# sohmandal/classpose

Measured on AMD Instinct MI355X. Metric: wsi_tiles_per_sec, higher is better.
Workload: dtype bf16; 1 GPU; configs[1]: synthetic 10000x10000 WSI (1936 tiles), tile 256 / overlap 32, conic 7 classes, ViT-L ClassTransformer depth 24 random-init, batch 32 sub-tiles = 8 WSI tiles/step, every step a distinct batch of the rank's shard (tiles sharded k % n_gpus, at most 256 distinct batches resident, longer runs wrap) streamed pinned host -> hipMemcpyAsync inside the timed region (the reader decodes ahead int; slide=10000, tile=256, overlap=32, batch_subtiles=32, distinct_batches=143, records_gathered=2048, decode_ahead_batches_at_t0=4, device_resident_batches_at_t0=1

## Files before the change

classpose_amd/csrc/cpx_attn2w.hip:

```cpp
#include "cpx_internal.h"
#include <type_traits>

namespace {
typedef __attribute__((ext_vector_type(8))) __bf16 bf16x8;
typedef __attribute__((ext_vector_type(8))) _Float16 f16x8;
typedef __attribute__((ext_vector_type(16))) float f32x16;
typedef __attribute__((ext_vector_type(2))) float f32x2;
typedef __attribute__((ext_vector_type(2))) __bf16 bf16x2;
typedef __attribute__((ext_vector_type(2))) _Float16 f16x2;
typedef __attribute__((ext_vector_type(4))) unsigned u32x4;

template <bool F16>
__device__ __forceinline__ f32x16 mfma32(const u32x4 &a, const u32x4 &b, f32x16 c) {
    if constexpr (F16)
        return __builtin_amdgcn_mfma_f32_32x32x16_f16(__builtin_bit_cast(f16x8, a), __builtin_bit_cast(f16x8, b), c, 0, 0, 0);
    else
        return __builtin_amdgcn_mfma_f32_32x32x16_bf16(__builtin_bit_cast(bf16x8, a), __builtin_bit_cast(bf16x8, b), c, 0, 0, 0);
}
template <bool F16>
__device__ __forceinline__ unsigned pack2(float lo, float hi) {
    f32x2 v = {lo, hi};
    if constexpr (F16) return __builtin_bit_cast(unsigned, __builtin_convertvector(v, f16x2));
    else return __builtin_bit_cast(unsigned, __builtin_convertvector(v, bf16x2));
}
__device__ __forceinline__ int pi_perm(int r) { return (r & ~12) | ((r & 4) << 1) | ((r & 8) >> 1); }
template <int OFF>
__device__ __forceinline__ u32x4 a2w_read128(unsigned addr) {
    u32x4 v;
    asm volatile("ds_read_b128 %0, %1 offset:%2" : "=v"(v) : "v"(addr), "n"(OFF));
    return v;
}
}

#define A2W_THREADS 256
#define A2W_SLOT 8192
#define A2W_G_LD 66
#define A2W_LDS_BYTES (4 * A2W_SLOT + 8 * 32 * A2W_G_LD * 2)
static_assert(A2W_LDS_BYTES <= 80 * 1024, "two workgroups per CU");

template <bool F16>
__global__ void __launch_bounds__(A2W_THREADS, 2) k_attention2w(const unsigned short *__restrict__ qkv,
                                                                 const unsigned short *__restrict__ vT,
                                                                 const unsigned short *__restrict__ relh,
                                                                 const unsigned short *__restrict__ relw,
                                                                 unsigned short *__restrict__ out, int xcd_order) {
    extern __shared__ __attribute__((aligned(16))) char a2w_smem[];
    const int tid = threadIdx.x, lane = tid & 63;
    const int wave = __builtin_amdgcn_readfirstlane(tid >> 6);
    const int r = lane & 31, h2 = lane >> 5;
    const int lin = (blockIdx.z * gridDim.y + blockIdx.y) * gridDim.x + blockIdx.x;
    int rg = blockIdx.x, head = blockIdx.y, s = blockIdx.z;
    if (xcd_order) {
        const int j = lin >> 3, pair = (j >> 2) * 8 + (lin & 7);
        rg = j & 3; head = pair & 15; s = pair >> 4;
    }
    const int qh0 = rg * 8 + wave * 2;
    const size_t tok0 = (size_t)s * 1024;
    const int kkey = tid >> 3, vd = tid >> 2;
    const unsigned short *ksrc = qkv + (tok0 + kkey) * 3072 + 1024 + head * 64 + (((tid & 7) ^ ((kkey >> 1) & 7)) * 8);
    const unsigned short *vsrc = vT + (((size_t)s * 16 + head) * 64 + vd) * 1024 + (((tid & 3) ^ ((vd >> 2) & 3)) * 8);
    char *dma_dst = a2w_smem + wave * 1024;
    auto issue = [&](int kh) {
        char *d = dma_dst + (kh & 3) * A2W_SLOT;
        __builtin_amdgcn_global_load_lds((const __attribute__((address_space(1))) void *)(ksrc + (size_t)kh * 32 * 3072),
                                         (__attribute__((address_space(3))) void *)d, 16, 0, 0);
        __builtin_amdgcn_global_load_lds((const __attribute__((address_space(1))) void *)(vsrc + kh * 32),
                                         (__attribute__((address_space(3))) void *)(d + 4096), 16, 0, 0);
    };
    issue(0); issue(1); issue(2);

    u32x4 qf[2][4];
#pragma unroll
    for (int c = 0; c < 2; ++c) {
        const unsigned short *qrow = qkv + (tok0 + (qh0 + c) * 32 + r) * 3072 + head * 64;
#pragma unroll
        for (int ks = 0; ks < 4; ++ks) qf[c][ks] = *reinterpret_cast<const u32x4 *>(qrow + 16 * ks + 8 * h2);
    }
    f32x16 GW[2];
#pragma unroll
    for (int c = 0; c < 2; ++c) {
        _Float16 *G = reinterpret_cast<_Float16 *>(a2w_smem + 4 * A2W_SLOT) + (wave * 2 + c) * 32 * A2W_G_LD;
        auto compute_G = [&](const unsigned short *table) {
#pragma unroll
            for (int jb = 0; jb < 2; ++jb) {
                f32x16 acc;
#pragma unroll
                for (int i = 0; i < 16; ++i) acc[i] = 0.f;
#pragma unroll
                for (int ks = 0; ks < 4; ++ks) {
                    const u32x4 tf = *reinterpret_cast<const u32x4 *>(table + (jb * 32 + r) * 64 + 16 * ks + 8 * h2);
                    acc = mfma32<F16>(tf, qf[c][ks], acc);
                }
#pragma unroll
                for (int i = 0; i < 16; ++i) G[r * A2W_G_LD + jb * 32 + (i & 3) + 8 * (i >> 2) + 4 * h2] = (_Float16)acc[i];
            }
        };
        compute_G(relw);
#pragma unroll
        for (int i = 0; i < 16; ++i) GW[c][i] = (float)G[r * A2W_G_LD + (r - pi_perm((i & 3) + 8 * (i >> 2) + 4 * h2) + 31)];
        compute_G(relh);
    }
    asm volatile("s_waitcnt vmcnt(0) lgkmcnt(0)" ::: "memory");
    __builtin_amdgcn_s_barrier();

    const unsigned lds0 = (unsigned)(size_t)(__attribute__((address_space(3))) char *)a2w_smem;
    const int krow = pi_perm(r);
    unsigned ka[4], va[4];
#pragma unroll
    for (int ks = 0; ks < 4; ++ks) ka[ks] = lds0 + (unsigned)(krow * 128 + (((2 * ks + h2) ^ ((krow >> 1) & 7)) * 16));
#pragma unroll
    for (int db = 0; db < 2; ++db)
#pragma unroll
        for (int st = 0; st < 2; ++st) {
            const int d = db * 32 + r;
            va[db * 2 + st] = lds0 + 4096u + (unsigned)(d * 64 + (((2 * st + h2) ^ ((d >> 2) & 3)) * 16));
        }
    unsigned gaddr[2];
#pragma unroll
    for (int c = 0; c < 2; ++c)
        gaddr[c] = lds0 + 4u * A2W_SLOT + (unsigned)((((wave * 2 + c) * 32 + r) * A2W_G_LD + qh0 + c + 31) * 2);

    u32x4 kf[4], vf[4];
    unsigned ghb[2];
    kf[0] = a2w_read128<0>(ka[0]); kf[1] = a2w_read128<0>(ka[1]);
    kf[2] = a2w_read128<0>(ka[2]); kf[3] = a2w_read128<0>(ka[3]);
    asm volatile("ds_read_u16 %0, %1" : "=v"(ghb[0]) : "v"(gaddr[0]));
    asm volatile("ds_read_u16 %0, %1" : "=v"(ghb[1]) : "v"(gaddr[1]));
    asm volatile("s_waitcnt lgkmcnt(0)" : "+v"(kf[0]), "+v"(kf[1]), "+v"(kf[2]), "+v"(kf[3]), "+v"(ghb[0]), "+v"(ghb[1])::"memory");
    f32x16 S[2], O0[2], O1[2];
    S[0] = mfma32<F16>(kf[0], qf[0][0], GW[0]);
    S[0] = mfma32<F16>(kf[1], qf[0][1], S[0]);
    S[0] = mfma32<F16>(kf[2], qf[0][2], S[0]);
    S[0] = mfma32<F16>(kf[3], qf[0][3], S[0]);
#pragma unroll
    for (int c = 0; c < 2; ++c)
#pragma unroll
        for (int i = 0; i < 16; ++i) { O0[c][i] = 0.f; O1[c][i] = 0.f; }
    float m_run[2] = {-1e30f, -1e30f}, l_run[2] = {0.f, 0.f};
    u32x4 pf[2][2];
    const float cexp = 0.125f * 1.44269504088896340736f;
    constexpr float HEADROOM = F16 ? 3.0f : 6.0f;
    using std::integral_constant;

    auto softmax = [&](auto chain_tag, unsigned gh_bits) {
        constexpr int C = decltype(chain_tag)::value;
        const float gh = (float)__builtin_bit_cast(_Float16, (unsigned short)gh_bits);
        float p[16];
        unsigned pk[8];
        {
            const float off = (gh - m_run[C]) * cexp;
#pragma unroll
            for (int i = 0; i < 16; ++i) p[i] = __builtin_amdgcn_exp2f(__builtin_fmaf(S[C][i], cexp, off));
#pragma unroll
            for (int j = 0; j < 8; ++j) pk[j] = pack2<F16>(p[2 * j], p[2 * j + 1]);
        }
        float a0 = (p[0] + p[1]) + (p[2] + p[3]), a1 = (p[4] + p[5]) + (p[6] + p[7]);
        float a2 = (p[8] + p[9]) + (p[10] + p[11]), a3 = (p[12] + p[13]) + (p[14] + p[15]);
        if (__builtin_expect(__any(((pk[0] | pk[1] | pk[2]) | (pk[3] | pk[4] | pk[5]) | (pk[6] | pk[7])) & 0x40004000u), 0)) {
            float mx = __builtin_fmaxf(__builtin_fmaxf(S[C][0], S[C][1]), S[C][2]);
#pragma unroll
            for (int i = 3; i < 15; i += 2) mx = __builtin_fmaxf(__builtin_fmaxf(mx, S[C][i]), S[C][i + 1]);
            mx = __builtin_fmaxf(mx, S[C][15]);
            mx = __builtin_fmaxf(mx, __shfl_xor(mx, 32)) + gh + HEADROOM / cexp;
            const float m_new = __builtin_fmaxf(m_run[C], mx);
            const float alpha = __builtin_amdgcn_exp2f((m_run[C] - m_new) * cexp);
            m_run[C] = m_new;
            l_run[C] *= alpha;
#pragma unroll
            for (int i = 0; i < 16; ++i) { O0[C][i] *= alpha; O1[C][i] *= alpha; }
            const float off = (gh - m_run[C]) * cexp;
#pragma unroll
            for (int i = 0; i < 16; ++i) p[i] = __builtin_amdgcn_exp2f(__builtin_fmaf(S[C][i], cexp, off));
#pragma unroll
            for (int j = 0; j < 8; ++j) pk[j] = pack2<F16>(p[2 * j], p[2 * j + 1]);
            a0 = (p[0] + p[1]) + (p[2] + p[3]); a1 = (p[4] + p[5]) + (p[6] + p[7]);
            a2 = (p[8] + p[9]) + (p[10] + p[11]); a3 = (p[12] + p[13]) + (p[14] + p[15]);
        }
        l_run[C] += (a0 + a1) + (a2 + a3);
        pf[C][0] = (u32x4){pk[0], pk[1], pk[2], pk[3]};
        pf[C][1] = (u32x4){pk[4], pk[5], pk[6], pk[7]};
    };
    auto pv = [&](auto chain_tag) {
        constexpr int C = decltype(chain_tag)::value;
        O0[C] = mfma32<F16>(vf[0], pf[C][0], O0[C]);
        O1[C] = mfma32<F16>(vf[2], pf[C][0], O1[C]);
        O0[C] = mfma32<F16>(vf[1], pf[C][1], O0[C]);
        O1[C] = mfma32<F16>(vf[3], pf[C][1], O1[C]);
    };
    auto qk = [&](auto chain_tag) {
        constexpr int C = decltype(chain_tag)::value;
        S[C] = mfma32<F16>(kf[0], qf[C][0], GW[C]);
        S[C] = mfma32<F16>(kf[1], qf[C][1], S[C]);
        S[C] = mfma32<F16>(kf[2], qf[C][2], S[C]);
        S[C] = mfma32<F16>(kf[3], qf[C][3], S[C]);
    };
    using C0 = integral_constant<int, 0>;
    using C1 = integral_constant<int, 1>;

    auto tile = [&](const int kh, auto slot_tag, auto next_tag, auto tail_tag, auto first_tag) {
        constexpr int SL = decltype(slot_tag)::value, SN = decltype(next_tag)::value, TAIL = decltype(tail_tag)::value;
        constexpr bool FIRST = decltype(first_tag)::value;
        if constexpr (TAIL < 2) asm volatile("s_waitcnt vmcnt(2)" ::: "memory");
        else asm volatile("s_waitcnt vmcnt(0)" ::: "memory");
        __builtin_amdgcn_s_barrier();
        if constexpr (TAIL == 0) issue(kh + 3);
        unsigned ghn[2] = {0u, 0u};
        if constexpr (TAIL < 3) {
            asm volatile("ds_read_u16 %0, %1" : "=v"(ghn[0]) : "v"(gaddr[0] - 2u * (unsigned)(kh + 1)));
            asm volatile("ds_read_u16 %0, %1" : "=v"(ghn[1]) : "v"(gaddr[1] - 2u * (unsigned)(kh + 1)));
        }
        __builtin_amdgcn_sched_barrier(0);
        qk(C1{});
        if constexpr (!FIRST) pv(C1{});
        softmax(C0{}, ghb[0]);
        __builtin_amdgcn_sched_barrier(0);
        if constexpr (TAIL < 3) {
            kf[0] = a2w_read128<SN * A2W_SLOT>(ka[0]); kf[1] = a2w_read128<SN * A2W_SLOT>(ka[1]);
            kf[2] = a2w_read128<SN * A2W_SLOT>(ka[2]); kf[3] = a2w_read128<SN * A2W_SLOT>(ka[3]);
        }
        vf[0] = a2w_read128<SL * A2W_SLOT>(va[0]); vf[1] = a2w_read128<SL * A2W_SLOT>(va[1]);
        vf[2] = a2w_read128<SL * A2W_SLOT>(va[2]); vf[3] = a2w_read128<SL * A2W_SLOT>(va[3]);
        asm volatile("s_waitcnt lgkmcnt(0)" : "+v"(kf[0]), "+v"(kf[1]), "+v"(kf[2]), "+v"(kf[3]), "+v"(vf[0]), "+v"(vf[1]),
                     "+v"(vf[2]), "+v"(vf[3]), "+v"(ghn[0]), "+v"(ghn[1])::"memory");
        __builtin_amdgcn_sched_barrier(0);
        if constexpr (TAIL < 3) qk(C0{});
        pv(C0{});
        softmax(C1{}, ghb[1]);
        __builtin_amdgcn_sched_barrier(0);
        ghb[0] = ghn[0]; ghb[1] = ghn[1];
    };
    using T0 = integral_constant<int, 0>;
    using NF = std::false_type;
    tile(0, integral_constant<int, 0>{}, integral_constant<int, 1>{}, T0{}, std::true_type{});
    tile(1, integral_constant<int, 1>{}, integral_constant<int, 2>{}, T0{}, NF{});
    tile(2, integral_constant<int, 2>{}, integral_constant<int, 3>{}, T0{}, NF{});
    tile(3, integral_constant<int, 3>{}, integral_constant<int, 0>{}, T0{}, NF{});
    for (int kh0 = 4; kh0 < 28; kh0 += 4) {
        tile(kh0 + 0, integral_constant<int, 0>{}, integral_constant<int, 1>{}, T0{}, NF{});
        tile(kh0 + 1, integral_constant<int, 1>{}, integral_constant<int, 2>{}, T0{}, NF{});
        tile(kh0 + 2, integral_constant<int, 2>{}, integral_constant<int, 3>{}, T0{}, NF{});
        tile(kh0 + 3, integral_constant<int, 3>{}, integral_constant<int, 0>{}, T0{}, NF{});
    }
    tile(28, integral_constant<int, 0>{}, integral_constant<int, 1>{}, T0{}, NF{});
    tile(29, integral_constant<int, 1>{}, integral_constant<int, 2>{}, integral_constant<int, 1>{}, NF{});
    tile(30, integral_constant<int, 2>{}, integral_constant<int, 3>{}, integral_constant<int, 2>{}, NF{});
    tile(31, integral_constant<int, 3>{}, integral_constant<int, 0>{}, integral_constant<int, 3>{}, NF{});
    pv(C1{});

#pragma unroll
    for (int c = 0; c < 2; ++c) {
        const float l_tot = l_run[c] + __shfl_xor(l_run[c], 32);
        const float inv = 1.0f / l_tot;
        unsigned short *orow = out + (tok0 + (qh0 + c) * 32 + r) * 1024 + head * 64;
#pragma unroll
        for (int db = 0; db < 2; ++db)
#pragma unroll
            for (int g4 = 0; g4 < 4; g4 += 2) {
                const f32x16 &O = db ? O1[c] : O0[c];
                unsigned ax = pack2<F16>(O[4 * g4 + 0] * inv, O[4 * g4 + 1] * inv), ay = pack2<F16>(O[4 * g4 + 2] * inv, O[4 * g4 + 3] * inv);
                unsigned bx = pack2<F16>(O[4 * g4 + 4] * inv, O[4 * g4 + 5] * inv), by = pack2<F16>(O[4 * g4 + 6] * inv, O[4 * g4 + 7] * inv);
                const auto rx = __builtin_amdgcn_permlane32_swap(ax, bx, false, false);
                const auto ry = __builtin_amdgcn_permlane32_swap(ay, by, false, false);
                *reinterpret_cast<uint4 *>(orow + db * 32 + 8 * g4 + 8 * h2) = make_uint4(rx[0], ry[0], rx[1], ry[1]);
            }
    }
}

int cpx_attention2w_launch(int dtype, const void *qkv, const void *vT, const void *rel_h, const void *rel_w,
                           int n_subtiles, void *out, int xcd_order, hipStream_t s) {
    static CpxOncePerDevice once;
    once([] {
        (void)hipFuncSetAttribute((const void *)k_attention2w<true>, hipFuncAttributeMaxDynamicSharedMemorySize, A2W_LDS_BYTES);
        (void)hipFuncSetAttribute((const void *)k_attention2w<false>, hipFuncAttributeMaxDynamicSharedMemorySize, A2W_LDS_BYTES);
    });
    const dim3 grid(4, 16, n_subtiles);
    if (dtype == CPX_DT_F16)
        hipLaunchKernelGGL((k_attention2w<true>), grid, dim3(A2W_THREADS), A2W_LDS_BYTES, s, (const unsigned short *)qkv,
                           (const unsigned short *)vT, (const unsigned short *)rel_h, (const unsigned short *)rel_w,
                           (unsigned short *)out, xcd_order);
    else
        hipLaunchKernelGGL((k_attention2w<false>), grid, dim3(A2W_THREADS), A2W_LDS_BYTES, s, (const unsigned short *)qkv,
                           (const unsigned short *)vT, (const unsigned short *)rel_h, (const unsigned short *)rel_w,
                           (unsigned short *)out, xcd_order);
    CPX_CHECK_LAUNCH();
    return CPX_OK;
}
```

Measured before the change: 374.2 tiles/s.

## Stage rel-pos tables via LDS DMA and batch G prologue MFMAs

The attention prologue now DMAs the relh/relw tables into LDS alongside the first K/V slot instead of each wave loading them from global memory. It computes all eight relative-position G tiles in one batched MFMA block, writes them with packed ds_write_b64 stores, and reads the diagonal GW terms back with fixed-offset ds_read_u16. Issue of the second and third K/V prefetch is deferred until after the MFMAs, with hand-tuned vmcnt waits. The aim is to shorten the serialized prologue latency. In exchange it uses more LDS (G stride 68, extra table slots) and relies on fragile manual waitcnt counts.

```diff
diff --git a/classpose_amd/csrc/cpx_attn2w.hip b/classpose_amd/csrc/cpx_attn2w.hip
--- a/classpose_amd/csrc/cpx_attn2w.hip
+++ b/classpose_amd/csrc/cpx_attn2w.hip
@@ -9,6 +9,7 @@
 typedef __attribute__((ext_vector_type(2))) __bf16 bf16x2;
 typedef __attribute__((ext_vector_type(2))) _Float16 f16x2;
 typedef __attribute__((ext_vector_type(4))) unsigned u32x4;
+typedef __attribute__((ext_vector_type(2))) unsigned u32x2;
 
 template <bool F16>
 __device__ __forceinline__ f32x16 mfma32(const u32x4 &a, const u32x4 &b, f32x16 c) {
@@ -30,12 +31,36 @@
     asm volatile("ds_read_b128 %0, %1 offset:%2" : "=v"(v) : "v"(addr), "n"(OFF));
     return v;
 }
+template <int OFF>
+__device__ __forceinline__ unsigned a2w_read16(unsigned addr) {
+    unsigned v;
+    asm volatile("ds_read_u16 %0, %1 offset:%2" : "=v"(v) : "v"(addr), "n"(OFF));
+    return v;
+}
+template <int OFF>
+__device__ __forceinline__ void a2w_write64(unsigned addr, unsigned lo, unsigned hi) {
+    const u32x2 v = {lo, hi};
+    asm volatile("ds_write_b64 %0, %1 offset:%2" ::"v"(addr), "v"(v), "n"(OFF) : "memory");
+}
+template <int OFF>
+__device__ __forceinline__ u32x4 a2w_gload128(const unsigned short *p) {
+    u32x4 v;
+    asm volatile("global_load_dwordx4 %0, %1, off offset:%2" : "=v"(v) : "v"(p), "n"(OFF) : "memory");
+    return v;
+}
+__device__ __forceinline__ void a2w_dma16(const unsigned short *src, char *dst) {
+    __builtin_amdgcn_global_load_lds((const __attribute__((address_space(1))) void *)src,
+                                     (__attribute__((address_space(3))) void *)dst, 16, 0, 0);
+}
 }
 
 #define A2W_THREADS 256
 #define A2W_SLOT 8192
-#define A2W_G_LD 66
-#define A2W_LDS_BYTES (4 * A2W_SLOT + 8 * 32 * A2W_G_LD * 2)
+#define A2W_TW (3 * A2W_SLOT)
+#define A2W_TH (4 * A2W_SLOT)
+#define A2W_G_OFF (5 * A2W_SLOT)
+#define A2W_G_LD 68
+#define A2W_LDS_BYTES (A2W_G_OFF + 8 * 32 * A2W_G_LD * 2)
 static_assert(A2W_LDS_BYTES <= 80 * 1024, "two workgroups per CU");
 
 template <bool F16>
@@ -62,48 +87,101 @@
     char *dma_dst = a2w_smem + wave * 1024;
     auto issue = [&](int kh) {
         char *d = dma_dst + (kh & 3) * A2W_SLOT;
-        __builtin_amdgcn_global_load_lds((const __attribute__((address_space(1))) void *)(ksrc + (size_t)kh * 32 * 3072),
-                                         (__attribute__((address_space(3))) void *)d, 16, 0, 0);
-        __builtin_amdgcn_global_load_lds((const __attribute__((address_space(1))) void *)(vsrc + kh * 32),
-                                         (__attribute__((address_space(3))) void *)(d + 4096), 16, 0, 0);
-    };
-    issue(0); issue(1); issue(2);
-
+        a2w_dma16(ksrc + (size_t)kh * 32 * 3072, d);
+        a2w_dma16(vsrc + kh * 32, d + 4096);
+    };
+    const unsigned lds0 = (unsigned)(size_t)(__attribute__((address_space(3))) char *)a2w_smem;
+
+    {
+        const int toff = kkey * 64 + (((tid & 7) ^ ((kkey >> 1) & 7)) * 8);
+        a2w_dma16(relw + toff, dma_dst + A2W_TW);
+        a2w_dma16(relw + toff + 32 * 64, dma_dst + A2W_TW + 4096);
+        a2w_dma16(relh + toff, dma_dst + A2W_TH);
+        a2w_dma16(relh + toff + 32 * 64, dma_dst + A2W_TH + 4096);
+    }
     u32x4 qf[2][4];
 #pragma unroll
     for (int c = 0; c < 2; ++c) {
-        const unsigned short *qrow = qkv + (tok0 + (qh0 + c) * 32 + r) * 3072 + head * 64;
-#pragma unroll
-        for (int ks = 0; ks < 4; ++ks) qf[c][ks] = *reinterpret_cast<const u32x4 *>(qrow + 16 * ks + 8 * h2);
-    }
+        const unsigned short *qrow = qkv + (tok0 + (qh0 + c) * 32 + r) * 3072 + head * 64 + 8 * h2;
+        qf[c][0] = a2w_gload128<0>(qrow); qf[c][1] = a2w_gload128<32>(qrow);
+        qf[c][2] = a2w_gload128<64>(qrow); qf[c][3] = a2w_gload128<96>(qrow);
+    }
+    issue(0);
+    asm volatile("s_waitcnt vmcnt(10)" ::: "memory");
+    __builtin_amdgcn_s_barrier();
+    u32x4 tw[2][4], th[2][4];
+    {
+        unsigned ta[4];
+#pragma unroll
+        for (int ks = 0; ks < 4; ++ks) ta[ks] = lds0 + (unsigned)(r * 128 + (((2 * ks + h2) ^ ((r >> 1) & 7)) * 16));
+#pragma unroll
+        for (int ks = 0; ks < 4; ++ks) {
+            tw[0][ks] = a2w_read128<A2W_TW>(ta[ks]); tw[1][ks] = a2w_read128<A2W_TW + 4096>(ta[ks]);
+            th[0][ks] = a2w_read128<A2W_TH>(ta[ks]); th[1][ks] = a2w_read128<A2W_TH + 4096>(ta[ks]);
+        }
+    }
+    asm volatile("s_waitcnt vmcnt(2) lgkmcnt(0)"
+                 : "+v"(qf[0][0]), "+v"(qf[0][1]), "+v"(qf[0][2]), "+v"(qf[0][3]), "+v"(qf[1][0]), "+v"(qf[1][1]), "+v"(qf[1][2]),
+                   "+v"(qf[1][3]), "+v"(tw[0][0]), "+v"(tw[0][1]), "+v"(tw[0][2]), "+v"(tw[0][3]), "+v"(tw[1][0]), "+v"(tw[1][1]),
+                   "+v"(tw[1][2]), "+v"(tw[1][3]), "+v"(th[0][0]), "+v"(th[0][1]), "+v"(th[0][2]), "+v"(th[0][3]), "+v"(th[1][0]),
+                   "+v"(th[1][1]), "+v"(th[1][2]), "+v"(th[1][3])::"memory");
+    f32x16 gacc[2][2][2];
+#pragma unroll
+    for (int t = 0; t < 2; ++t)
+#pragma unroll
+        for (int jb = 0; jb < 2; ++jb)
+#pragma unroll
+            for (int c = 0; c < 2; ++c) {
+                f32x16 acc;
+#pragma unroll
+                for (int i = 0; i < 16; ++i) acc[i] = 0.f;
+#pragma unroll
+                for (int ks = 0; ks < 4; ++ks) acc = mfma32<F16>(t ? th[jb][ks] : tw[jb][ks], qf[c][ks], acc);
+                gacc[t][c][jb] = acc;
+            }
+    __builtin_amdgcn_sched_barrier(0);
+    issue(1); issue(2);
+    unsigned gwb[2][16];
+    auto store_G = [&](int t) {
+#pragma unroll
+        for (int c = 0; c < 2; ++c) {
+            const unsigned ga = lds0 + A2W_G_OFF + (unsigned)((((wave * 2 + c) * 32 + r) * A2W_G_LD + 4 * h2) * 2);
+#pragma unroll
+            for (int jb = 0; jb < 2; ++jb) {
+                const f32x16 &acc = gacc[t][c][jb];
+                a2w_write64<0>(ga + jb * 64, pack2<true>(acc[0], acc[1]), pack2<true>(acc[2], acc[3]));
+                a2w_write64<16>(ga + jb * 64, pack2<true>(acc[4], acc[5]), pack2<true>(acc[6], acc[7]));
+                a2w_write64<32>(ga + jb * 64, pack2<true>(acc[8], acc[9]), pack2<true>(acc[10], acc[11]));
+                a2w_write64<48>(ga + jb * 64, pack2<true>(acc[12], acc[13]), pack2<true>(acc[14], acc[15]));
+            }
+        }
+    };
+    store_G(0);
+#pragma unroll
+    for (int c = 0; c < 2; ++c) {
+        const unsigned ga = lds0 + A2W_G_OFF + (unsigned)((((wave * 2 + c) * 32 + r) * A2W_G_LD + r + 8 - 8 * h2) * 2);
+        gwb[c][0] = a2w_read16<46>(ga); gwb[c][1] = a2w_read16<44>(ga); gwb[c][2] = a2w_read16<42>(ga); gwb[c][3] = a2w_read16<40>(ga);
+        gwb[c][4] = a2w_read16<38>(ga); gwb[c][5] = a2w_read16<36>(ga); gwb[c][6] = a2w_read16<34>(ga); gwb[c][7] = a2w_read16<32>(ga);
+        gwb[c][8] = a2w_read16<14>(ga); gwb[c][9] = a2w_read16<12>(ga); gwb[c][10] = a2w_read16<10>(ga); gwb[c][11] = a2w_read16<8>(ga);
+        gwb[c][12] = a2w_read16<6>(ga); gwb[c][13] = a2w_read16<4>(ga); gwb[c][14] = a2w_read16<2>(ga); gwb[c][15] = a2w_read16<0>(ga);
+    }
+    asm volatile("s_waitcnt lgkmcnt(0)"
+                 : "+v"(gwb[0][0]), "+v"(gwb[0][1]), "+v"(gwb[0][2]), "+v"(gwb[0][3]), "+v"(gwb[0][4]), "+v"(gwb[0][5]), "+v"(gwb[0][6]),
+                   "+v"(gwb[0][7]), "+v"(gwb[0][8]), "+v"(gwb[0][9]), "+v"(gwb[0][10]), "+v"(gwb[0][11]), "+v"(gwb[0][12]),
+                   "+v"(gwb[0][13]), "+v"(gwb[0][14]), "+v"(gwb[0][15])::"memory");
+    asm volatile(""
+                 : "+v"(gwb[1][0]), "+v"(gwb[1][1]), "+v"(gwb[1][2]), "+v"(gwb[1][3]), "+v"(gwb[1][4]), "+v"(gwb[1][5]), "+v"(gwb[1][6]),
+                   "+v"(gwb[1][7]), "+v"(gwb[1][8]), "+v"(gwb[1][9]), "+v"(gwb[1][10]), "+v"(gwb[1][11]), "+v"(gwb[1][12]),
+                   "+v"(gwb[1][13]), "+v"(gwb[1][14]), "+v"(gwb[1][15])::"memory");
+    store_G(1);
     f32x16 GW[2];
 #pragma unroll
-    for (int c = 0; c < 2; ++c) {
-        _Float16 *G = reinterpret_cast<_Float16 *>(a2w_smem + 4 * A2W_SLOT) + (wave * 2 + c) * 32 * A2W_G_LD;
-        auto compute_G = [&](const unsigned short *table) {
-#pragma unroll
-            for (int jb = 0; jb < 2; ++jb) {
-                f32x16 acc;
-#pragma unroll
-                for (int i = 0; i < 16; ++i) acc[i] = 0.f;
-#pragma unroll
-                for (int ks = 0; ks < 4; ++ks) {
-                    const u32x4 tf = *reinterpret_cast<const u32x4 *>(table + (jb * 32 + r) * 64 + 16 * ks + 8 * h2);
-                    acc = mfma32<F16>(tf, qf[c][ks], acc);
-                }
-#pragma unroll
-                for (int i = 0; i < 16; ++i) G[r * A2W_G_LD + jb * 32 + (i & 3) + 8 * (i >> 2) + 4 * h2] = (_Float16)acc[i];
-            }
-        };
-        compute_G(relw);
-#pragma unroll
-        for (int i = 0; i < 16; ++i) GW[c][i] = (float)G[r * A2W_G_LD + (r - pi_perm((i & 3) + 8 * (i >> 2) + 4 * h2) + 31)];
-        compute_G(relh);
-    }
-    asm volatile("s_waitcnt vmcnt(0) lgkmcnt(0)" ::: "memory");
+    for (int c = 0; c < 2; ++c)
+#pragma unroll
+        for (int i = 0; i < 16; ++i) GW[c][i] = (float)__builtin_bit_cast(_Float16, (unsigned short)gwb[c][i]);
+    asm volatile("s_waitcnt vmcnt(4) lgkmcnt(0)" ::: "memory");
     __builtin_amdgcn_s_barrier();
 
-    const unsigned lds0 = (unsigned)(size_t)(__attribute__((address_space(3))) char *)a2w_smem;
     const int krow = pi_perm(r);
     unsigned ka[4], va[4];
 #pragma unroll
@@ -118,7 +196,7 @@
     unsigned gaddr[2];
 #pragma unroll
     for (int c = 0; c < 2; ++c)
-        gaddr[c] = lds0 + 4u * A2W_SLOT + (unsigned)((((wave * 2 + c) * 32 + r) * A2W_G_LD + qh0 + c + 31) * 2);
+        gaddr[c] = lds0 + A2W_G_OFF + (unsigned)((((wave * 2 + c) * 32 + r) * A2W_G_LD + qh0 + c + 31) * 2);
 
     u32x4 kf[4], vf[4];
     unsigned ghb[2];
```

After: 377.1 tiles/s, median of 6. No clear change (+0.8%).
